# Apokleos/kata-xpu-device-plugin

Measured on NVIDIA H100. Metric: pci.ids parse GB/s (x1000 text + 2^20-key join); device lookups/s reported beside it, higher is better.
Workload: dtype u8

## Files before the change

### kata-xpu-device-plugin_b200/csrc/api.cu

```cuda
#include <algorithm>
#include <cstdlib>
#include <new>
#include <vector>

#include "internal.cuh"
#include "pciids5.cu"
#include "finalize.cuh"
#include "small.cuh"
#include "scan.cuh"

void kx_exchange_destroy(kxpu_ctx *ctx);

static const char *kx_err_names[] = {
    "ok", "invalid argument", "CUDA error", "no sm_90 GPU available", "output buffer too small",
    "table capacity exceeded", "NCCL / peer exchange unavailable or failed", "input outside the supported domain", "out of memory"};

extern "C" const char *kxpu_strerror(int32_t status) {
    int i = -status;
    if (i < 0 || i > 8) return "unknown status";
    return kx_err_names[i];
}

extern "C" const char *kxpu_last_error(kxpu_ctx *ctx) {
    if (!ctx) return "null ctx";
// ... 270 lines not shown
    t->dev.slots = (KxSlot *)(b + L.o_slots);
    t->dev.vendor_first = (unsigned long long *)(b + L.o_vfirst);
    t->dev.trunc = (unsigned long long *)(b + L.o_trunc);
    t->dev.counters = (uint32_t *)(b + L.o_counters);
    t->dev.cap = cap;
    t->dev.shift = t->shift;
    t->dev.max_keys = cap / 2;
    t->range_words = (unsigned long long *)(b + L.o_range);
    t->row_key = (uint32_t *)(b + L.o_row_key);
    t->row_line = (unsigned long long *)(b + L.o_row_line);
    t->row_anchor = (unsigned long long *)(b + L.o_row_anchor);
    t->row_name_off = (uint32_t *)(b + L.o_row_noff);
    t->row_name_len = (uint32_t *)(b + L.o_row_nlen);
    t->blob = b + L.o_blob;
    t->blob_cap = blob_cap;
    t->rows_cap = cap + 1;
    *out = t;
    return KXPU_OK;
}

void kx_table_release(kxpu_ctx *ctx, kxpu_table *t) {
    if (!t) return;
    if (t->arena.p) {
        if (ctx->pool.size() >= 4) {
            cudaStreamSynchronize(ctx->stream);
            cudaFree(ctx->pool.front().p);
            ctx->pool.erase(ctx->pool.begin());
        }
        arena_reset(ctx, t->arena);
        ctx->pool.push_back(t->arena);
    }
    delete t;
}

uint32_t kx_initial_blob_cap(kxpu_ctx *ctx, size_t n) {
    const uint32_t by_text = (uint32_t)std::min<size_t>(std::max<size_t>(n, 256), 4u << 20);
    return ctx->blob_hint > by_text ? ctx->blob_hint : by_text;
}

bool kx_grow_cap(uint32_t *cap, bool table_full) {
    if (*cap >= (1u << 28)) return false;
    const uint32_t sh = table_full ? 4u : 2u;
    *cap = (*cap >> (28u - sh)) ? (1u << 28) : (*cap << sh);
    return true;
}

void kx_note_table_size(kxpu_ctx *ctx, uint32_t nkeys, uint32_t blob_used, uint32_t blob_cap) {
    uint32_t ideal = 1u << 16;
    while (ideal < (1u << 28) && ideal / 2 < nkeys + nkeys / 8) ideal <<= 1;
    ctx->cap_hint = ideal;
    ctx->blob_hint = blob_cap > (4u << 20) && blob_used > (2u << 20) ? blob_cap : 0u;
}

int32_t kx_launch_parse(kxpu_ctx *ctx, kxpu_table *t, const uint8_t *d_text, size_t n, unsigned long long base,
                        unsigned long long carry_in, const KxXaHook *xa) {
    using namespace kxparse;
    const uint32_t num_chunks = (uint32_t)((n + CW - 1) / CW);
    kxparse5::Params5 P;
    memset(&P, 0, sizeof P);
    if (xa) { P.xa_on = 1; P.xa_done = xa->done; P.xa = xa->p; }
    if (num_chunks == 0) {
        if (xa) {
            P.tab = t->dev;
            P.task_ctas = 0;
            kxparse5::resolve_chunks_kernel<<<kxparse5::XA_CTAS, kxparse5::RES_WARPS * 32, 0, ctx->stream>>>(P);
            KX_LAUNCHED(ctx);
            KX_CUDA(ctx, cudaGetLastError());
        }
        return KXPU_OK;
    }
    P.text = d_text; P.n = n; P.base = base; P.num_chunks = num_chunks;
    P.tma_limit = n >= (size_t)STG_BYTES ? (uint32_t)((n - STG_BYTES) / CW) + 1u : 0u;
    static int per_sm = 0;
    const size_t smem = sizeof(kxparse5::WarpSmem5) * WARPS;
    if (per_sm == 0) {
        cudaOccupancyMaxActiveBlocksPerMultiprocessor(&per_sm, kxparse5::parse_kernel_v5, NT, smem);
        if (per_sm < 1) per_sm = 1;
    }
    const uint32_t wave_warps = (uint32_t)per_sm * ctx->sm_count * WARPS;
    P.rch = std::min<uint32_t>(std::max<uint32_t>(num_chunks / (wave_warps * 8u), 1u), kxparse5::RCH5_MAX);
    if (ctx->force_rch) P.rch = (uint32_t)ctx->force_rch;
    P.num_ranges = (num_chunks + P.rch - 1) / P.rch;
    P.range_state = t->range_words;
    P.range_carry = t->range_words + P.num_ranges;
    P.lead = (uint32_t *)(t->range_words + 2 * P.num_ranges);
    P.tasks = P.lead + P.num_ranges;
    P.tab = t->dev; P.carry_in = carry_in;
    uint32_t grid = (uint32_t)per_sm * ctx->sm_count;
    const uint32_t need = (P.num_ranges + WARPS - 1) / WARPS;
    if (grid > need) grid = need;
    {
        KxTimer tm(ctx, KXPU_T_PARSE);
        kxparse5::parse_kernel_v5<<<grid, NT, smem, ctx->stream>>>(P);
        KX_LAUNCHED(ctx);
    }
    {
        KxTimer tr(ctx, KXPU_T_RESOLVE);
        kxparse5::resolve_ranges_kernel<<<(P.num_ranges + 255u) / 256u, 256, 0, ctx->stream>>>(P);
        KX_LAUNCHED(ctx);
        const uint32_t rgrid = std::min<uint32_t>(4u * ctx->sm_count, (num_chunks + kxparse5::RES_WARPS - 1) / kxparse5::RES_WARPS);
        P.task_ctas = rgrid;
        kxparse5::resolve_chunks_kernel<<<rgrid + (xa ? kxparse5::XA_CTAS : 0u), kxparse5::RES_WARPS * 32, 0, ctx->stream>>>(P);
        KX_LAUNCHED(ctx);
    }
    KX_CUDA(ctx, cudaGetLastError());
    return KXPU_OK;
}

int32_t kx_launch_trunc(kxpu_ctx *ctx, kxpu_table *t, const uint8_t *d_text, size_t n, unsigned long long base) {
    kxparse::trunc_kernel<<<1, 1024, 0, ctx->stream>>>(d_text, n, base, t->dev.trunc, t->dev.counters);
    KX_LAUNCHED(ctx);
    KX_CUDA(ctx, cudaGetLastError());
    return KXPU_OK;
}

int32_t kx_launch_finalize(kxpu_ctx *ctx, kxpu_table *t, const uint8_t *d_text, size_t n, unsigned long long base,
                           const kxx::MinView *mv, const kxx::WaitSpec *wait, const KxSlabOut *slab) {
    kxparse::FinalizeParams F;
    memset(&F, 0, sizeof F);
    if (wait) F.wait = *wait;
    F.text = d_text; F.n = n; F.base = base; F.tab = t->dev;
    if (mv) F.mv = *mv;
    else { F.mv.a = t->dev.vendor_first; F.mv.stride = 0; F.mv.n = 1; F.mv.trunc1 = t->dev.trunc; }
    F.row_key = t->row_key; F.row_line = t->row_line; F.row_anchor = t->row_anchor;
    F.row_name_off = t->row_name_off; F.row_name_len = t->row_name_len;
    F.blob = t->blob; F.blob_cap = t->blob_cap;
    if (slab) {
        F.slab_rows = reinterpret_cast<kxx::SlabRow *>(slab->rows); F.slab_rows_cap = slab->rows_cap;
        F.blob = slab->blob; F.blob_cap = slab->blob_cap;
        F.tail = slab->tail;
    }
    KxTimer tm(ctx, KXPU_T_FINALIZE);
    F.scan_w = t->cap >= (1u << 19) ? 32u : 8u;
    if (ctx->force_scan_w) F.scan_w = (uint32_t)ctx->force_scan_w;
    const unsigned batches = (t->cap + 1 + F.scan_w - 1) / F.scan_w;
    const unsigned grid = std::min<unsigned>((batches + kxparse::SF_WARPS - 1) / kxparse::SF_WARPS, 8u * ctx->sm_count);
    kxparse::select_finalize_kernel<<<grid, kxparse::SF_WARPS * 32, 0, ctx->stream>>>(F);
    KX_LAUNCHED(ctx);
    KX_CUDA(ctx, cudaGetLastError());
    return KXPU_OK;
}

static unsigned join_ctas(kxpu_ctx *ctx, size_t n) { return (unsigned)std::min<size_t>((n + 255) / 256, (size_t)ctx->sm_count * 32); }

int32_t kx_launch_lookup(kxpu_ctx *ctx, kxpu_table *t, const uint32_t *d_keys, size_t n, int32_t *d_rows) {
    if (n == 0) return KXPU_OK;
    KxTimer tm(ctx, KXPU_T_LOOKUP);
    kxparse::lookup_kernel<<<join_ctas(ctx, n), 256, 0, ctx->stream>>>(d_keys, n, t->dev.slots, t->cap, t->shift, d_rows);
    KX_LAUNCHED(ctx);
    KX_CUDA(ctx, cudaGetLastError());
    return KXPU_OK;
}

static int32_t kx_launch_rows_names_join(kxpu_ctx *ctx, kxpu_table *t, const uint8_t *d_text, size_t n, const uint32_t *d_keys,
                                         size_t nq, int32_t *d_rows) {
    using namespace kxparse;
    FinalizeParams F;
    memset(&F, 0, sizeof F);
    F.text = d_text; F.n = n; F.base = 0; F.tab = t->dev;
    F.mv.a = t->dev.vendor_first; F.mv.stride = 0; F.mv.n = 1; F.mv.trunc1 = t->dev.trunc;
    F.row_key = t->row_key; F.row_line = t->row_line; F.row_anchor = t->row_anchor;
    F.row_name_off = t->row_name_off; F.row_name_len = t->row_name_len;
    F.blob = t->blob; F.blob_cap = t->blob_cap;
    KxTimer tm(ctx, KXPU_T_FINALIZE);
    select_rows_kernel<<<(t->cap + SF_WARPS * 32) / (SF_WARPS * 32), SF_WARPS * 32, 0, ctx->stream>>>(F);
    KX_LAUNCHED(ctx);
    const uint32_t want = (t->cap / 2 + SF_CTA_ROWS - 1) / SF_CTA_ROWS;
    const unsigned name_ctas = std::max<unsigned>(1u, std::min<unsigned>(want, 8u * ctx->sm_count));
    const unsigned grid = name_ctas + (nq ? join_ctas(ctx, nq) : 0u);
    names_join_kernel<<<grid, SF_WARPS * 32, 0, ctx->stream>>>(F, name_ctas, d_keys, nq, d_rows);
    KX_LAUNCHED(ctx);
    KX_CUDA(ctx, cudaGetLastError());
    return KXPU_OK;
}

struct KxJoin {
    const uint32_t *d_keys;
    size_t n;
    int32_t *d_rows;
    int32_t *h_rows;
    const uint8_t *src_text;
};

static void *kx_mapped_host(const void *p) {
    if (!p) return nullptr;
    cudaPointerAttributes at;
    if (cudaPointerGetAttributes(&at, p) != cudaSuccess) { cudaGetLastError(); return nullptr; }
    return at.type == cudaMemoryTypeHost ? at.devicePointer : nullptr;
}

static uint32_t small_text_chunks(kxpu_ctx *ctx) {
    if (ctx->small_chunks < 0) {
        int coop = 0, per_sm = 0;
        cudaDeviceGetAttribute(&coop, cudaDevAttrCooperativeLaunch, ctx->device);
        cudaFuncSetAttribute(kxsmall::small_load_kernel, cudaFuncAttributeMaxDynamicSharedMemorySize, kxparse::WARPS * kxparse::STG_BYTES);
        cudaOccupancyMaxActiveBlocksPerMultiprocessor(&per_sm, kxsmall::small_load_kernel, kxparse::NT, kxparse::WARPS * kxparse::STG_BYTES);
        cudaGetLastError();
        ctx->small_chunks = (coop && !ctx->no_small) ? per_sm * ctx->sm_count * kxparse::WARPS : 0;
    }
    return (uint32_t)ctx->small_chunks;
}

static int32_t launch_small(kxpu_ctx *ctx, kxpu_table *t, const uint8_t *d_text, size_t n, const KxJoin *join) {
    using namespace kxparse;
    kxsmall::SmallParams P;
    memset(&P, 0, sizeof P);
    P.text = d_text; P.n = n;
    P.num_chunks = (uint32_t)((n + CW - 1) / CW);
    P.tma_limit = n >= (size_t)STG_BYTES ? (uint32_t)((n - STG_BYTES) / CW) + 1u : 0u;
    P.state = t->range_words;
    FinalizeParams &F = P.F;
    F.text = d_text; F.n = n; F.base = 0; F.tab = t->dev;
    F.mv.a = t->dev.vendor_first; F.mv.stride = 0; F.mv.n = 1; F.mv.trunc1 = t->dev.trunc;
    F.row_key = t->row_key; F.row_line = t->row_line; F.row_anchor = t->row_anchor;
    F.row_name_off = t->row_name_off; F.row_name_len = t->row_name_len;
    F.blob = t->blob; F.blob_cap = t->blob_cap;
    if (join) { P.keys = join->d_keys; P.nq = join->n; P.rows_out = join->d_rows; }
    if (join && join->src_text) { P.text_src = join->src_text; P.h_ctl = ctx->h_ctl; }
    void *args[] = {&P};
    const unsigned grid = std::max<unsigned>((P.num_chunks + WARPS - 1) / WARPS, (unsigned)(ctx->small_chunks / WARPS));
    F.scan_w = 8u;
    while (F.scan_w < 32u && (size_t)(t->cap + 1 + F.scan_w - 1) / F.scan_w > (size_t)grid * SF_WARPS) F.scan_w *= 2u;
    if (ctx->force_scan_w) F.scan_w = (uint32_t)ctx->force_scan_w;
// ... 37 lines not shown
                fprintf(stderr, " %u: %lld/%lld/%lld/%lld |", c, tw[c * 4], tw[c * 4 + 1], tw[c * 4 + 2], tw[c * 4 + 3]);
            }
            const unsigned mid = wv[wv.size() / 2].second;
            fprintf(stderr, " median %u: %lld/%lld/%lld/%lld", mid, tw[mid * 4], tw[mid * 4 + 1], tw[mid * 4 + 2], tw[mid * 4 + 3]);
            const long long *tf = h.data() + (size_t)grid * 8 + (size_t)P.num_chunks * 4;
            static const char *fn[7] = {"scan", "rounds", "sync1+claim", "sync2", "names out+rows", "long lines", "shift+sync3"};
            fprintf(stderr, "\n   names phase per CTA (thread 0), cycles min/avg/max:");
            for (int k = 0; k < 7; k++) {
                long long mn = 1ll << 62, mx = 0, sum = 0, cnt = 0;
                for (unsigned b = 0; b < grid; b++) {
                    const long long t1 = tf[b * 8 + k], t0 = k ? tf[b * 8 + k - 1] : h[b * 8 + 4];
                    if (!t1 || !t0) continue;
                    const long long d = t1 - t0;
                    mn = std::min(mn, d); mx = std::max(mx, d); sum += d; cnt++;
                }
                if (cnt) fprintf(stderr, " %s %lld/%lld/%lld |", fn[k], mn, sum / cnt, mx);
            }
        }
        fprintf(stderr, "\n");
    }
    return KXPU_OK;
}

static int32_t kx_build_table_join(kxpu_ctx *ctx, const uint8_t *d_text, size_t n, kxpu_table **out, const KxJoin *join) {
    if ((reinterpret_cast<uintptr_t>(d_text) & 15u) != 0) {
        KX_SET_ERR(ctx, "device text pointer must be 16-byte aligned");
        return KXPU_E_INVALID;
    }
    if (n >= (1ull << 44)) return KXPU_E_UNSUPPORTED;
    uint32_t cap = ctx->cap_hint;
    while (cap > (1u << 16) && (size_t)cap / 2 > n / 6 + 1) cap >>= 1;
    uint32_t blob_cap = kx_initial_blob_cap(ctx, n);
    const uint32_t num_chunks = (uint32_t)((n + kxparse::CW - 1) / kxparse::CW);
    bool have_trunc = false;
    for (int attempt = 0; attempt < 12; attempt++) {
        kxpu_table *t = nullptr;
        int32_t rc = kx_table_acquire(ctx, cap, blob_cap, num_chunks, &t);
        if (rc != KXPU_OK) return rc;
        const bool small_path = num_chunks > 0 && num_chunks <= small_text_chunks(ctx) && !have_trunc;
        if (small_path) {
            rc = launch_small(ctx, t, d_text, n, join);
        } else {
            if (join && join->src_text && attempt == 0) cudaMemcpyAsync(const_cast<uint8_t *>(d_text), join->src_text, n, cudaMemcpyDefault, ctx->stream);
            rc = kx_launch_parse(ctx, t, d_text, n, 0, 0, nullptr);
            if (rc == KXPU_OK && have_trunc) rc = kx_launch_trunc(ctx, t, d_text, n, 0);
            if (rc == KXPU_OK)
                rc = join ? kx_launch_rows_names_join(ctx, t, d_text, n, join->d_keys, join->n, join->d_rows)
                          : kx_launch_rows_names_join(ctx, t, d_text, n, nullptr, 0, nullptr);
        }
        if (rc != KXPU_OK) { kx_table_release(ctx, t); return rc; }
        const bool zero_copy = small_path && join && join->src_text;
        if (!zero_copy) {
            if (join && join->h_rows && join->n) cudaMemcpyAsync(join->h_rows, join->d_rows, join->n * 4, cudaMemcpyDeviceToHost, ctx->stream);
            cudaMemcpyAsync(ctx->h_ctl, t->dev.counters, KX_C_COUNT * 4, cudaMemcpyDeviceToHost, ctx->stream);
        }
        cudaError_t e = cudaStreamSynchronize(ctx->stream);
        if (e != cudaSuccess) {
            KX_SET_ERR(ctx, "parse/finalize failed: %s", cudaGetErrorString(e));
            kx_table_release(ctx, t);
            return KXPU_E_CUDA;
        }
        const uint32_t *h = ctx->h_ctl;
        if (h[KX_C_OVERFLOW] || h[KX_C_NKEYS] > t->dev.max_keys) {
            kx_table_release(ctx, t);
            if (!kx_grow_cap(&cap, h[KX_C_OVERFLOW] != 0)) return KXPU_E_CAPACITY;
            continue;
        }
        if (h[KX_C_NEED_TRUNC] == 2u) {
            kx_table_release(ctx, t);
            have_trunc = true;
            continue;
        }
        if (h[KX_C_BLOB_OVERFLOW]) {
            kx_table_release(ctx, t);
            if ((size_t)blob_cap >= n) return KXPU_E_CAPACITY;
            blob_cap = (uint32_t)std::min<size_t>(std::max<size_t>(n, 256), (size_t)blob_cap * 8);
            continue;
        }
        t->n_rows = h[KX_C_NSEL];
        t->blob_used = h[KX_C_BLOB_CURSOR];
        kx_note_table_size(ctx, h[KX_C_NKEYS], t->blob_used, blob_cap);
        *out = t;
        return KXPU_OK;
    }
    return KXPU_E_CAPACITY;
}

extern "C" int32_t kxpu_pciids_load_device(kxpu_ctx *ctx, const void *d_text, size_t n, kxpu_table **out) {
    KX_ENTER(ctx);
    if (!out || (!d_text && n)) return KXPU_E_INVALID;
    kx_clear_timings(ctx);
    return kx_build_table_join(ctx, (const uint8_t *)d_text, n, out, nullptr);
}

extern "C" int32_t kxpu_pciids_join_device(kxpu_ctx *ctx, const void *d_text, size_t n, const uint32_t *d_keys, size_t nq,
                                           int32_t *d_rows_out, kxpu_table **out) {
    KX_ENTER(ctx);
    if (!out || (!d_text && n) || (nq && (!d_keys || !d_rows_out))) return KXPU_E_INVALID;
    kx_clear_timings(ctx);
    const KxJoin j{d_keys, nq, d_rows_out, nullptr, nullptr};
    return kx_build_table_join(ctx, (const uint8_t *)d_text, n, out, &j);
}

static int32_t stage_reserve(kxpu_ctx *ctx, size_t bytes) {
    if (bytes <= ctx->d_stage_bytes) return KXPU_OK;
    if (ctx->d_stage) {
        cudaStreamSynchronize(ctx->stream);
// ... 167 lines not shown
```

### kata-xpu-device-plugin_b200/csrc/common.cuh

```cuda
#pragma once
#include <cuda_runtime.h>
#include <stdint.h>
#include <stdio.h>
#include <string.h>

#include <mutex>
#include <vector>

#include "../../include/kxpu.h"

constexpr int KX_MAX_RANKS = 16;


struct KxArena {
    void *p = nullptr;
    size_t bytes = 0;
    uint32_t cap = 0, blob_cap = 0;
    size_t range_bytes = 0;
};

struct KxExchange;
struct kxpu_multi;

struct kxpu_ctx {
// ... 37 lines not shown
            KX_SET_ERR(ctx, "%s:%d %s -> %s", __FILE__, __LINE__, #call, cudaGetErrorString(e__)); \
            return KXPU_E_CUDA;                                                             \
        }                                                                                   \
    } while (0)

#define KX_LAUNCHED(ctx) ((ctx)->launches++)

struct KxTimer {
    kxpu_ctx *c;
    int idx;
    bool open = true;
    KxTimer(kxpu_ctx *ctx, int i) : c(ctx), idx(i) {
        open = c->stage_timing;
        if (open) cudaEventRecord(c->ev[2 * i], c->stream);
    }
    void stop() {
        if (open) { cudaEventRecord(c->ev[2 * idx + 1], c->stream); c->ev_used[idx] = true; open = false; }
    }
    ~KxTimer() { stop(); }
};

static inline void kx_clear_timings(kxpu_ctx *c) { memset(c->ev_used, 0, sizeof(c->ev_used)); }

unsigned long long *kx_scan_state(kxpu_ctx *ctx, size_t words);
uint32_t kx_next_epoch(kxpu_ctx *ctx);

int32_t kx_rule_drivers(kxpu_ctx *ctx, const kxpu_xpu_rule *rules, size_t n_rules, unsigned long long drv[][4]);

void kx_pcie_parse(cudaStream_t st, const kxpu_devrec *recs, const kxpu_pcipath *paths, uint32_t n, unsigned long long *chain,
                   uint8_t *clen);

struct KxScratch {
    kxpu_ctx *c;
    std::vector<void *> ptrs;
    explicit KxScratch(kxpu_ctx *ctx) : c(ctx) {}
    cudaError_t alloc(void **p, size_t bytes) {
        cudaError_t e = cudaMallocAsync(p, bytes ? bytes : 16, c->stream);
        if (e == cudaSuccess) ptrs.push_back(*p);
        else *p = nullptr;
        return e;
    }
    ~KxScratch() {
        for (void *p : ptrs) cudaFreeAsync(p, c->stream);
    }
};

#ifdef __CUDACC__
__device__ __forceinline__ uint32_t kx_lane() { return threadIdx.x & 31u; }

__device__ __forceinline__ void kx_fence_gpu() { asm volatile("fence.acq_rel.gpu;" ::: "memory"); }
__device__ __forceinline__ void kx_fence_sys() { asm volatile("fence.acq_rel.sys;" ::: "memory"); }

__device__ __forceinline__ uint32_t kx_hash(uint32_t key) { return key * 0x9E3779B1u; }
#endif
```

### kata-xpu-device-plugin_b200/csrc/finalize.cuh

```cuda
#pragma once
#include "exchange.cuh"
#include "parse_common.cuh"

namespace kxparse {

constexpr unsigned long long MAX_TOKEN = 65536ull;

__global__ void __launch_bounds__(1024) trunc_kernel(const uint8_t *__restrict__ text, unsigned long long n,
                                                      unsigned long long base, unsigned long long *trunc_out, uint32_t *counters) {
    __shared__ unsigned long long s_first[1024], s_last[1024], s_bad[1024];
    const unsigned long long per = (n + 1023ull) / 1024ull;
    const unsigned long long lo = per * threadIdx.x, hi = lo + per < n ? lo + per : n;
    unsigned long long first = KX_NO_OFF, last = KX_NO_OFF, bad = KX_NO_OFF;
    for (unsigned long long i = lo; i < hi; i++) {
        if (text[i] == (uint8_t)'\n') {
            if (first == KX_NO_OFF) first = i;
            else if (i - last - 1 >= MAX_TOKEN && bad == KX_NO_OFF) bad = last + 1;
            last = i;
        }
    }
    s_first[threadIdx.x] = first; s_last[threadIdx.x] = last; s_bad[threadIdx.x] = bad;
    __syncthreads();
    if (threadIdx.x == 0) {
        unsigned long long prev_nl = KX_NO_OFF;
// ... 386 lines not shown
        }
        SF_MARK(5);
        {
            const uint32_t rem = qn - nvalid;
            if (nvalid != 0u && rem != 0u) {
                SfEntry e;
                if (lane < rem) e = q[nvalid + lane];
                __syncwarp();
                if (lane < rem) q[lane] = e;
                __syncwarp();
            }
            qn = rem;
        }
        __syncthreads();
        SF_MARK(6);
        if (!more) break;
    }
}

__global__ void __launch_bounds__(SF_WARPS * 32, 8) select_finalize_kernel(const FinalizeParams F) {
    kxx::wait_flags_cta(F.wait);
    select_finalize_body(F, F.scan_w);
    if (F.tail.on) {
        __syncthreads();
        if (threadIdx.x == 0) {
            kx_fence_sys();
            const uint32_t prev = atomicAdd(F.tail.done, 1u);
            if (prev == gridDim.x - 1u) {
                *F.tail.done = 0u;
                kx_fence_gpu();
                const volatile uint32_t *c = F.tab.counters;
                const uint32_t n_sel = c[KX_C_NSEL], blob_used = c[KX_C_BLOB_CURSOR];
                const bool over = c[KX_C_BLOB_OVERFLOW] || n_sel > F.tail.rows_cap || blob_used > F.tail.blob_cap;
                kxx::SlabHeader h;
                memset(&h, 0, sizeof h);
                h.n_rows = over ? 0u : n_sel;
                h.blob_bytes = over ? 0u : blob_used;
                h.status = over ? kxx::XS_SLAB_OVERFLOW : 0u;
                if (c[KX_C_OVERFLOW]) h.status |= kxx::XS_GROW | kxx::XS_FULL;
                if (c[KX_C_NKEYS] > F.tab.max_keys) h.status |= kxx::XS_GROW;
                h.nkeys = c[KX_C_NKEYS];
                *F.tail.header = h;
                kx_fence_sys();
                for (int k = 0; k < F.tail.tg.n; k++) *reinterpret_cast<volatile uint32_t *>(F.tail.tg.region[k] + F.tail.o_flag) = F.tail.epoch;
            }
        }
    }
}

constexpr uint32_t SF_CTA_ROWS = SF_WARPS * SF_BATCH;

__global__ void __launch_bounds__(SF_WARPS * 32) select_rows_kernel(const FinalizeParams F) {
    __shared__ uint32_t s_cnt[SF_WARPS], s_row0;
    if (sf_stand_back(F)) return;
    const uint32_t lane = threadIdx.x & 31u, wl = threadIdx.x >> 5;
    const uint32_t slot = blockIdx.x * blockDim.x + threadIdx.x;
    uint32_t key = 0;
    unsigned long long line = 0, anchor = 0;
    const bool valid = slot <= F.tab.cap && sf_slot_valid(F, slot, kxx::min_view_trunc(F.mv), key, line, anchor);
    const uint32_t vm = __ballot_sync(0xffffffffu, valid);
    if (lane == 0) s_cnt[wl] = (uint32_t)__popc(vm);
    __syncthreads();
    if (threadIdx.x == 0) {
        uint32_t rows = 0, blob0;
#pragma unroll
        for (int k = 0; k < SF_WARPS; k++) rows += s_cnt[k];
        sf_cta_claim(F, rows, 0u, s_row0, blob0);
    }
    __syncthreads();
    if (valid) {
        uint32_t row = s_row0 + (uint32_t)__popc(vm & ((1u << lane) - 1u));
        for (uint32_t k = 0; k < wl; k++) row += s_cnt[k];
        F.tab.slots[slot].row = (int32_t)row;
        F.row_key[row] = key; F.row_line[row] = line; F.row_anchor[row] = anchor;
    }
}

__device__ __forceinline__ void names_body(const FinalizeParams &F, uint32_t ctas) {
    __shared__ __align__(16) uint8_t s_raw[SF_WARPS][4][SF_WIN + 16];
    __shared__ uint8_t s_name[SF_WARPS][SF_BATCH][SF_WIN];
    __shared__ uint32_t s_bytes[SF_WARPS], s_blob0;
    const uint32_t lane = threadIdx.x & 31u, wl = threadIdx.x >> 5;
    const uint32_t n_rows = F.tab.counters[KX_C_NSEL];
    for (uint32_t c0 = blockIdx.x * SF_CTA_ROWS; c0 < n_rows; c0 += ctas * SF_CTA_ROWS) {
        const uint32_t r0 = c0 + wl * (uint32_t)SF_BATCH;
        const uint32_t nvalid = r0 < n_rows ? min(n_rows - r0, (uint32_t)SF_BATCH) : 0u;
        uint32_t my_len, slow_m;
        sf_name_batch(F, lane < nvalid ? F.row_line[r0 + lane] : 0ull, nvalid, s_raw[wl], s_name[wl], my_len, slow_m);
        const uint32_t len_r = (lane < nvalid && !((slow_m >> lane) & 1u)) ? my_len : 0u;
        const uint32_t incl = sf_incl_scan(len_r);
        const uint32_t wtot = __shfl_sync(0xffffffffu, incl, 31);
        if (lane == 0) s_bytes[wl] = wtot;
        __syncthreads();
        if (threadIdx.x == 0) {
            uint32_t bytes = 0, row0;
#pragma unroll
            for (int k = 0; k < SF_WARPS; k++) bytes += s_bytes[k];
            sf_cta_claim(F, 0u, bytes, row0, s_blob0);
        }
        __syncthreads();
        uint32_t blob0 = s_blob0;
        for (uint32_t k = 0; k < wl; k++) if (blob0 != 0xFFFFFFFFu) blob0 += s_bytes[k];
        const bool room = blob0 != 0xFFFFFFFFu;
        const uint32_t off_r = room ? blob0 + incl - len_r : 0u, len_w = room ? len_r : 0u;
        sf_names_out(F, s_name[wl], nvalid, len_w, off_r);
        if (lane < nvalid && !((slow_m >> lane) & 1u)) { F.row_name_off[r0 + lane] = off_r; F.row_name_len[r0 + lane] = len_w; }
        __syncwarp();
        for (uint32_t sm = slow_m; sm; sm &= sm - 1u) {
            const uint32_t r = (uint32_t)__ffs((int)sm) - 1u;
            uint32_t name_off, name_len;
            sf_long_name(F, F.row_line[r0 + r], &s_name[wl][0][0], name_off, name_len);
            if (lane == 0) { F.row_name_off[r0 + r] = name_off; F.row_name_len[r0 + r] = name_len; }
            __syncwarp();
        }
        __syncthreads();
    }
}

__global__ void __launch_bounds__(SF_WARPS * 32, 8) names_join_kernel(const FinalizeParams F, uint32_t name_ctas,
                                                                       const uint32_t *__restrict__ keys, size_t nq,
                                                                       int32_t *__restrict__ rows_out) {
    if (blockIdx.x < name_ctas) {
        names_body(F, name_ctas);
        return;
    }
    const size_t stride = (size_t)(gridDim.x - name_ctas) * blockDim.x;
    for (size_t i = (size_t)(blockIdx.x - name_ctas) * blockDim.x + threadIdx.x; i < nq; i += stride)
        rows_out[i] = table_probe(F.tab.slots, F.tab.cap, F.tab.shift, keys[i]);
}

__global__ void __launch_bounds__(256) lookup_kernel(const uint32_t *__restrict__ keys, size_t n, const KxSlot *__restrict__ slots,
                                                      uint32_t cap, uint32_t shift, int32_t *__restrict__ rows_out) {
    size_t i = (size_t)blockIdx.x * blockDim.x + threadIdx.x;
    const size_t stride = (size_t)gridDim.x * blockDim.x;
    for (; i < n; i += stride) rows_out[i] = table_probe(slots, cap, shift, keys[i]);
}

__global__ void __launch_bounds__(256) name_len_kernel(const int32_t *__restrict__ rows, size_t n,
                                                        const uint32_t *__restrict__ row_name_len, uint32_t n_rows,
                                                        uint32_t *__restrict__ lens) {
    size_t i = (size_t)blockIdx.x * blockDim.x + threadIdx.x;
    if (i < n) {
        int32_t r = rows[i];
        lens[i] = (r >= 0 && (uint32_t)r < n_rows) ? row_name_len[r] : 0u;
    }
}
__global__ void __launch_bounds__(256) name_copy_kernel(const int32_t *__restrict__ rows, size_t n,
                                                         const uint32_t *__restrict__ row_name_off,
                                                         const uint32_t *__restrict__ row_name_len, uint32_t n_rows,
                                                         const uint8_t *__restrict__ blob,
                                                         const uint32_t *__restrict__ offsets, uint8_t *__restrict__ out,
                                                         size_t cap) {
    size_t i = ((size_t)blockIdx.x * blockDim.x + threadIdx.x) >> 3;
    uint32_t sub = threadIdx.x & 7u;
    if (i >= n) return;
    int32_t r = rows[i];
    if (r < 0 || (uint32_t)r >= n_rows) return;
    uint32_t len = row_name_len[r], src = row_name_off[r], dst = offsets[i];
    if ((size_t)dst + len > cap) return;
    for (uint32_t k = sub; k < len; k += 8u) out[dst + k] = blob[src + k];
}

__global__ void __launch_bounds__(256) arena_reset_kernel(uint4 *ff, size_t n_ff16, uint32_t *counters) {
    const size_t i = (size_t)blockIdx.x * blockDim.x + threadIdx.x;
    const size_t stride = (size_t)gridDim.x * blockDim.x;
    for (size_t k = i; k < n_ff16; k += stride) ff[k] = make_uint4(0xffffffffu, 0xffffffffu, 0xffffffffu, 0xffffffffu);
    if (i < KX_C_COUNT) counters[i] = 0u;
}

}
```

### kata-xpu-device-plugin_b200/csrc/pciids5.cu

```cuda
#pragma once
#include "exchange.cuh"
#include "parse_common.cuh"

namespace kxparse5 {

using namespace kxparse;

constexpr int CPC5 = 3;
constexpr int STAGES5 = 2;
constexpr int CTAS5 = 2;
constexpr int COPY5 = CPC5 * CW + TRAIL;
constexpr int RCH5_MAX = CPC5 * STAGES5;
constexpr int RES_WARPS = 8;

struct WarpSmem5 {
    alignas(16) uint8_t stage[STAGES5][COPY5];
    alignas(8) unsigned long long bar[STAGES5];
};

struct Params5 {
    const uint8_t *text;
    unsigned long long n, base;
    uint32_t num_chunks;
    uint32_t tma_limit;
// ... 30 lines not shown
    }
}

__device__ __forceinline__ uint32_t tops_of(uint32_t lp, uint32_t mm) {
    uint32_t tm = 0;
    while (mm) {
        const uint32_t bit = mm & (0u - mm);
        mm ^= bit;
        const uint32_t c0 = lds8(lp + (31u - (uint32_t)__clz((int)bit)));
        if (c0 != 9u && c0 != 35u) tm |= bit;
    }
    return tm;
}

__device__ __forceinline__ void tops_of2(uint32_t lp0, uint32_t m0, uint32_t m1, uint32_t &t0, uint32_t &t1) {
    t0 = t1 = 0;
    while (m0 | m1) {
        const uint32_t b0 = m0 & (0u - m0), b1 = m1 & (0u - m1);
        m0 ^= b0;
        m1 ^= b1;
        const uint32_t c0 = lds8(lp0 + (31u - (uint32_t)__clz((int)b0)));
        const uint32_t c1 = lds8(lp0 + (uint32_t)HALF + (31u - (uint32_t)__clz((int)b1)));
        if (c0 != 9u && c0 != 35u) t0 |= b0;
        if (c1 != 9u && c1 != 35u) t1 |= b1;
    }
}

__device__ __forceinline__ uint32_t devs_of(uint32_t lp, uint32_t mm) {
    uint32_t km = 0;
    while (mm) {
        const uint32_t bit = mm & (0u - mm);
        mm ^= bit;
        const uint32_t a = lp + (31u - (uint32_t)__clz((int)bit));
        if (lds8(a) == 9u && lds8(a + 1u) != 9u) km |= bit;
    }
    return km;
}

__global__ void __launch_bounds__(NT, CTAS5) parse_kernel_v5(const Params5 P) {
    extern __shared__ __align__(128) uint8_t smem_raw[];
    WarpSmem5 *W = reinterpret_cast<WarpSmem5 *>(smem_raw);
    uint32_t lane = threadIdx.x & 31u;
    const uint32_t w = threadIdx.x >> 5;
    asm volatile("" : "+r"(lane));
    const uint32_t lt_mask = (1u << lane) - 1u;

    if (lane == 0) {
        for (int s = 0; s < STAGES5; s++) mbar_init(&W[w].bar[s], 1);
        asm volatile("fence.mbarrier_init.release.cluster;" ::: "memory");
    }
    uint32_t tk = 0;
    if (lane == 0) tk = atomicAdd(&P.tab.counters[KX_C_TICKET], 1u);
    uint32_t r = __shfl_sync(0xffffffffu, tk, 0);
    if (r >= P.num_ranges) return;

    uint32_t a_stage0 = smem_u32(smem_raw) + w * (uint32_t)sizeof(WarpSmem5);
    asm volatile("" : "+r"(a_stage0));
    const uint32_t a_bar0 = a_stage0 + (uint32_t)offsetof(WarpSmem5, bar);

    uint32_t k7f = 0x7f7f7f7fu, k0a = 0x0a0a0a0au, k80 = 0x80808080u;
    asm volatile("" : "+r"(k7f), "+r"(k0a), "+r"(k80));

    const unsigned long long pol = l2_evict_first_policy();
    const uint32_t rch = P.rch;
    auto copy_chunks = [](uint32_t cnt, uint32_t k) -> uint32_t {
        return cnt - k * (uint32_t)CPC5 < (uint32_t)CPC5 ? cnt - k * (uint32_t)CPC5 : (uint32_t)CPC5;
    };
    auto issue = [&](uint32_t g0, uint32_t m, uint32_t s) {
        if (g0 + m - 1u < P.tma_limit) {
            mbar_expect_tx_a(a_bar0 + 8u * s, m * (uint32_t)CW + (uint32_t)TRAIL);
            tma_load_a(a_stage0 + s * (uint32_t)COPY5, P.text + (unsigned long long)g0 * CW, m * (uint32_t)CW + (uint32_t)TRAIL, a_bar0 + 8u * s, pol);
        }
    };

    uint32_t phase_bits = 0, s = 0;
    uint32_t nfresh = 0;
    for (;;) {
        uint32_t tk2 = 0;
        if (lane == 0) tk2 = atomicAdd(&P.tab.counters[KX_C_TICKET], 1u);
        uint32_t rc_x = 0, rc_g = 0;
        if (r == 0u) {
            rc_x = LS_PUB | (((P.carry_in & CV_HAS_TOP) && (P.carry_in & CV_VOK)) ? (LS_TOP | LS_VOK) : 0u);
            rc_g = 0xffffffffu;
        }
        uint32_t lead = r == 0u ? 0u : rch;
        const bool table_dead = *reinterpret_cast<volatile uint32_t *>(&P.tab.counters[KX_C_OVERFLOW]) != 0u;
        const uint32_t gb = r * rch;
        const uint32_t cnt = P.num_chunks - gb < rch ? P.num_chunks - gb : rch;
        const uint32_t ncp = (cnt + (uint32_t)CPC5 - 1u) / (uint32_t)CPC5;
        if (lane == 0) {
            for (uint32_t j = 0; j < (uint32_t)STAGES5 && j < ncp; j++) issue(gb + j * (uint32_t)CPC5, copy_chunks(cnt, j), (s + j) % (uint32_t)STAGES5);
        }
        for (uint32_t k = 0; k < ncp; k++) {
            const uint32_t g0 = gb + k * (uint32_t)CPC5, m = copy_chunks(cnt, k);
            const bool by_tma = g0 + m - 1u < P.tma_limit;
            if (by_tma) {
                const uint32_t bar = a_bar0 + 8u * s, par = (phase_bits >> s) & 1u;
                while (!mbar_try_a(bar, par)) {
                }
                phase_bits ^= 1u << s;
            }
            for (uint32_t j = 0; j < m; j++) {
                const uint32_t i = k * (uint32_t)CPC5 + j;
                const uint32_t g = g0 + j;
                const uint32_t st = a_stage0 + s * (uint32_t)COPY5 + j * (uint32_t)CW;
                const unsigned long long cbase = P.base + (unsigned long long)g * CW;
                uint32_t n_rel = CW + 1;
// ... 92 lines not shown
                    const uint32_t l1 = __shfl_sync(0xffffffffu, linfo1, bal1 ? 31 - __clz((int)bal1) : 0);
                    const uint32_t last0 = bal0 ? l0 : base_info;
                    const uint32_t cin0 = s0 ? x0 : base_info;
                    const uint32_t cin1 = s1 ? x1 : last0;
                    last1 = bal1 ? l1 : last0;
                    if (cin0 != P_NONE && (cin0 >> 31))
                        fold_lines(P.tab, st, cbase, pre0, lane * 32u + 1u, ((cin0 >> 15) & 0xffffu) << 16, cbase + (cin0 & 0x7fffu), nfresh);
                    if (cin1 != P_NONE && (cin1 >> 31))
                        fold_lines(P.tab, st, cbase, pre1, (uint32_t)HALF + lane * 32u + 1u, ((cin1 >> 15) & 0xffffu) << 16, cbase + (cin1 & 0x7fffu), nfresh);
                    const uint32_t hw0 = cin0 == P_NONE ? pre0 : 0u;
                    const uint32_t hw1 = cin1 == P_NONE ? pre1 : 0u;
                    if (rc_x & LS_VOK) {
                        uint32_t key_hi = ((rc_x >> 12) & 0xffffu) << 16;
                        unsigned long long anchor = P.base + (unsigned long long)rc_g * CW + (rc_x & 0xfffu);
                        if (rc_g == 0xffffffffu) {
                            key_hi = ((uint32_t)(P.carry_in >> 44) & 0xffffu) << 16;
                            anchor = P.carry_in & CV_ANCHOR_MASK;
                        }
                        if ((hw0 | hw1) != 0u && P.tab.vendor_first[key_hi >> 16] >= anchor) {
                            fold_lines(P.tab, st, cbase, hw0, lane * 32u + 1u, key_hi, anchor, nfresh);
                            fold_lines(P.tab, st, cbase, hw1, (uint32_t)HALF + lane * 32u + 1u, key_hi, anchor, nfresh);
                        }
                    }
                    flush_fresh(P.tab, nfresh);
                }
                if (last1 != P_NONE) {
                    if (rc_x == 0u) lead = i + 1u;
                    rc_x = LS_PUB | LS_TOP | ((last1 >> 31) ? LS_VOK : 0u) | (((last1 >> 15) & 0xffffu) << 12) | (last1 & 0xfffu);
                    rc_g = g;
                }
                if ((bal0 | bal1) == 0u && n_rel > (uint32_t)CW && __reduce_or_sync(0xffffffffu, rawnl) == 0u && lane == 0)
                    atomicOr(&P.tab.counters[KX_C_LONGLINE_HINT], 1u);
                __syncwarp();
            }

            if (lane == 0 && k + (uint32_t)STAGES5 < ncp) issue(gb + (k + (uint32_t)STAGES5) * (uint32_t)CPC5, copy_chunks(cnt, k + (uint32_t)STAGES5), s);
            s = s == (uint32_t)STAGES5 - 1u ? 0u : s + 1u;
        }
        if (lane == 0) {
            unsigned long long v = ST_NONE;
            if (rc_x != 0u) {
                if (rc_g == 0xffffffffu)
                    v = ST_PREFIX | P.carry_in;
                else
                    v = ST_PREFIX | CV_HAS_TOP | ((rc_x & LS_VOK) ? CV_VOK : 0ull) | ((unsigned long long)((rc_x >> 12) & 0xffffu) << 44) |
                        ((P.base + (unsigned long long)rc_g * CW + (rc_x & 0xfffu)) & CV_ANCHOR_MASK);
            }
            P.range_state[r] = v;
            P.lead[r] = lead < cnt ? lead : cnt;
        }
        r = __shfl_sync(0xffffffffu, tk2, 0);
        if (r >= P.num_ranges) break;
    }
}

constexpr uint32_t XA_CTAS = 64;

__global__ void __launch_bounds__(256) resolve_ranges_kernel(const Params5 P) {
    const uint32_t rr = blockIdx.x * blockDim.x + threadIdx.x;
    const uint32_t lane = threadIdx.x & 31u;
    const uint32_t rr0 = rr - lane;
    if (rr0 >= P.num_ranges) return;
    const bool live = rr < P.num_ranges;
    const uint32_t nlead = live ? P.lead[rr] : 0u;
    const unsigned long long own = live ? P.range_state[rr] : ST_NONE;
    const uint32_t pm = __ballot_sync(0xffffffffu, (own & ST_MASK) == ST_PREFIX);
    const uint32_t below = pm & ((1u << lane) - 1u);
    const unsigned long long from_warp = __shfl_sync(0xffffffffu, own, below ? 31 - __clz((int)below) : 0);
    unsigned long long warp_in = 0;
    const uint32_t first_p = pm ? (uint32_t)__ffs((int)pm) - 1u : 32u;
    const bool want = __any_sync(0xffffffffu, nlead != 0u && lane <= first_p);
    if (want) {
        long long q0 = (long long)rr0 - 32;
        for (;;) {
            const long long q = q0 + lane;
            const unsigned long long sv = q >= 0 ? P.range_state[q] : (q == -1 ? (ST_PREFIX | P.carry_in) : ST_NONE);
            const uint32_t m = __ballot_sync(0xffffffffu, (sv & ST_MASK) == ST_PREFIX);
            if (m) {
                warp_in = __shfl_sync(0xffffffffu, sv, 31 - __clz((int)m));
                break;
            }
            q0 -= 32;
        }
    }
    const unsigned long long carry = (below ? from_warp : warp_in) & ~ST_MASK;
    const bool alive = nlead != 0u && (carry & CV_HAS_TOP) && (carry & CV_VOK) &&
                       P.tab.vendor_first[(uint32_t)(carry >> 44) & 0xffffu] >= (carry & CV_ANCHOR_MASK);
    const uint32_t mine = alive ? nlead : 0u;
    uint32_t incl = mine;
#pragma unroll
    for (int d = 1; d < 32; d <<= 1) {
        const uint32_t y = __shfl_up_sync(0xffffffffu, incl, d);
        if (lane >= (uint32_t)d) incl += y;
    }
    const uint32_t tot = __shfl_sync(0xffffffffu, incl, 31);
    uint32_t at0 = 0;
    if (lane == 0 && tot) at0 = atomicAdd(&P.tab.counters[KX_C_DEFER], tot);
    at0 = __shfl_sync(0xffffffffu, at0, 0);
    if (!alive) return;
    P.range_carry[rr] = carry;
    const uint32_t at = at0 + incl - mine;
    for (uint32_t j = 0; j < nlead; j++) P.tasks[at + j] = rr * P.rch + j;
}

__global__ void __launch_bounds__(RES_WARPS * 32) resolve_chunks_kernel(const Params5 P) {
    __shared__ __align__(16) uint8_t stg[RES_WARPS][STG_BYTES];
    __shared__ __align__(8) unsigned long long bars[RES_WARPS];
    __shared__ uint16_t plist[RES_WARPS][704];
    if (blockIdx.x >= P.task_ctas) {
        kxx::xa_push_slice(P.xa, (blockIdx.x - P.task_ctas) * blockDim.x + threadIdx.x, XA_CTAS * blockDim.x);
        __syncthreads();
        if (threadIdx.x == 0) {
            kx_fence_sys();
            const uint32_t prev = atomicAdd(P.xa_done, 1u);
            if (prev == XA_CTAS - 1u) {
                *P.xa_done = 0u;
                kx_fence_sys();
                kxx::xa_finish(P.xa);
            }
        }
        return;
    }
    const uint32_t lane = threadIdx.x & 31u, w = threadIdx.x >> 5;
    const uint32_t lt_mask = (1u << lane) - 1u;
    uint32_t k7f = 0x7f7f7f7fu, k0a = 0x0a0a0a0au, k80 = 0x80808080u;
    asm volatile("" : "+r"(k7f), "+r"(k0a), "+r"(k80));
    const uint32_t st = smem_u32(stg[w]), bar = smem_u32(&bars[w]);
    if (lane == 0) {
        mbar_init(&bars[w], 1);
        asm volatile("fence.mbarrier_init.release.cluster;" ::: "memory");
    }
    __syncwarp();
    const unsigned long long pol = l2_evict_first_policy();
    const uint32_t n_tasks = P.tab.counters[KX_C_DEFER];
    uint32_t par = 0, nfresh = 0;
    const bool small_tab = P.tab.cap <= (1u << 20);
    uint32_t it = 0;
    for (uint32_t t = blockIdx.x * RES_WARPS + w; t < n_tasks; t += P.task_ctas * RES_WARPS, it++) {
        if ((it & 3u) == 0u && *reinterpret_cast<volatile uint32_t *>(&P.tab.counters[KX_C_OVERFLOW]) != 0u) break;
        const uint32_t gg = P.tasks[t];
        uint32_t n_rel = CW + 1;
        if (gg < P.tma_limit) {
            if (lane == 0) {
                mbar_expect_tx_a(bar, STG_BYTES);
                tma_load_a(st, P.text + (unsigned long long)gg * CW, STG_BYTES, bar, pol);
            }
            while (!mbar_try_a(bar, par)) {
            }
            par ^= 1u;
        } else {
            n_rel = stage_chunk_manual(P.text, P.n, gg, lane, stg[w]);
        }
        const unsigned long long cc = P.range_carry[gg / P.rch];
        const uint32_t key_hi = ((uint32_t)(cc >> 44) & 0xffffu) << 16;
        const unsigned long long anchor = cc & CV_ANCHOR_MASK;
        uint32_t kh[2], th[2], rawnl;
        chunk_masks(st, lane, n_rel, k7f, k0a, k80, kh, th, rawnl);
        const uint32_t bal0 = __ballot_sync(0xffffffffu, th[0] != 0u);
        const uint32_t bal1 = __ballot_sync(0xffffffffu, th[1] != 0u);
        const uint32_t pre0 = kh[0] & ~th[0] & (th[0] ? (th[0] & (0u - th[0])) - 1u : 0xffffffffu);
        const uint32_t pre1 = kh[1] & ~th[1] & (th[1] ? (th[1] & (0u - th[1])) - 1u : 0xffffffffu);
        const unsigned long long cbase = P.base + (unsigned long long)gg * CW;
        const uint32_t m0 = (bal0 & lt_mask) == 0u ? pre0 : 0u;
        const uint32_t m1 = (bal0 == 0u && (bal1 & lt_mask) == 0u) ? pre1 : 0u;
        const uint32_t mine = (uint32_t)__popc(m0) + (uint32_t)__popc(m1);
        uint32_t incl = mine;
#pragma unroll
        for (int d = 1; d < 32; d <<= 1) {
            const uint32_t y = __shfl_up_sync(0xffffffffu, incl, d);
            if (lane >= (uint32_t)d) incl += y;
        }
        const uint32_t total = __shfl_sync(0xffffffffu, incl, 31);
        {
            uint32_t idx = incl - mine;
            for (uint32_t m = m0; m; m &= m - 1u) plist[w][idx++] = (uint16_t)(lane * 32u + 1u + (uint32_t)__ffs((int)m) - 1u);
            for (uint32_t m = m1; m; m &= m - 1u) plist[w][idx++] = (uint16_t)((uint32_t)HALF + lane * 32u + 1u + (uint32_t)__ffs((int)m) - 1u);
        }
        __syncwarp();
        if (small_tab) {
            for (uint32_t i = lane; i < total; i += 64u) {
                uint32_t d0, d1 = 0;
                const uint32_t p0 = plist[w][i], p1 = i + 32u < total ? plist[w][i + 32u] : 0u;
                bool v0 = hex4_swar(lds32_unaligned(st + p0 + 1u), d0);
                bool v1 = i + 32u < total && hex4_swar(lds32_unaligned(st + p1 + 1u), d1);
                uint32_t q0 = p0, q1 = p1;
                if (!v0 && v1) { d0 = d1; q0 = p1; v0 = true; v1 = false; }
// ... 16 lines not shown
```

### kata-xpu-device-plugin_b200/csrc/table.cuh

```cuda
#pragma once
#include "common.cuh"

#define KX_EMPTY_KEY 0xFFFFFFFFu
#define KX_NO_OFF 0xFFFFFFFFFFFFFFFFull

#define KX_C_TICKET 0
#define KX_C_DEFER 1
#define KX_C_GRIDBAR 2
#define KX_C_NKEYS 32
#define KX_C_NSEL 33
#define KX_C_BLOB_CURSOR 64
#define KX_C_OVERFLOW 96
#define KX_C_LONGLINE_HINT 97
#define KX_C_NROWS 98
#define KX_C_BLOB_OVERFLOW 99
#define KX_C_NEED_TRUNC 100
#define KX_C_XSTATUS 101
#define KX_C_XROWS 102
#define KX_C_XBLOB 103
#define KX_C_XMAXKEYS 104
#define KX_C_COUNT 128

struct __align__(32) KxSlot {
    uint32_t key;
    int32_t row;
    unsigned long long min_line;
    unsigned long long min_anchor;
    unsigned long long spare;
};

struct KxTableDev {
    KxSlot *slots;
    unsigned long long *vendor_first;
    uint32_t *counters;
    unsigned long long *trunc;
    uint32_t cap;
    uint32_t shift;
    uint32_t max_keys;
};
```

Baseline: 2687.

## Chain parse/resolve/finalize kernels with PDL and write counters to host from device

```diff
diff --git a/kata-xpu-device-plugin_b200/csrc/api.cu b/kata-xpu-device-plugin_b200/csrc/api.cu
--- a/kata-xpu-device-plugin_b200/csrc/api.cu
+++ b/kata-xpu-device-plugin_b200/csrc/api.cu
@@ -346,6 +346,23 @@
     ctx->blob_hint = blob_cap > (4u << 20) && blob_used > (2u << 20) ? blob_cap : 0u;
 }
 
+template <typename... KArgs, typename... Args>
+static cudaError_t kx_launch_pdl(kxpu_ctx *ctx, void (*kernel)(KArgs...), unsigned grid, unsigned block, size_t smem, Args &&...args) {
+    cudaLaunchAttribute at[1];
+    at[0].id = cudaLaunchAttributeProgrammaticStreamSerialization;
+    at[0].val.programmaticStreamSerializationAllowed = 1;
+    cudaLaunchConfig_t cfg = {};
+    cfg.gridDim = dim3(grid);
+    cfg.blockDim = dim3(block);
+    cfg.dynamicSmemBytes = smem;
+    cfg.stream = ctx->stream;
+    cfg.attrs = at;
+    cfg.numAttrs = 1;
+    const cudaError_t e = cudaLaunchKernelEx(&cfg, kernel, std::forward<Args>(args)...);
+    KX_LAUNCHED(ctx);
+    return e;
+}
+
 int32_t kx_launch_parse(kxpu_ctx *ctx, kxpu_table *t, const uint8_t *d_text, size_t n, unsigned long long base,
                         unsigned long long carry_in, const KxXaHook *xa) {
     using namespace kxparse;
@@ -390,12 +407,10 @@
     }
     {
         KxTimer tr(ctx, KXPU_T_RESOLVE);
-        kxparse5::resolve_ranges_kernel<<<(P.num_ranges + 255u) / 256u, 256, 0, ctx->stream>>>(P);
-        KX_LAUNCHED(ctx);
+        KX_CUDA(ctx, kx_launch_pdl(ctx, kxparse5::resolve_ranges_kernel, (P.num_ranges + 255u) / 256u, 256u, 0, P));
         const uint32_t rgrid = std::min<uint32_t>(4u * ctx->sm_count, (num_chunks + kxparse5::RES_WARPS - 1) / kxparse5::RES_WARPS);
         P.task_ctas = rgrid;
-        kxparse5::resolve_chunks_kernel<<<rgrid + (xa ? kxparse5::XA_CTAS : 0u), kxparse5::RES_WARPS * 32, 0, ctx->stream>>>(P);
-        KX_LAUNCHED(ctx);
+        KX_CUDA(ctx, kx_launch_pdl(ctx, kxparse5::resolve_chunks_kernel, rgrid + (xa ? kxparse5::XA_CTAS : 0u), kxparse5::RES_WARPS * 32u, 0, P));
     }
     KX_CUDA(ctx, cudaGetLastError());
     return KXPU_OK;
@@ -457,12 +472,11 @@
     F.row_name_off = t->row_name_off; F.row_name_len = t->row_name_len;
     F.blob = t->blob; F.blob_cap = t->blob_cap;
     KxTimer tm(ctx, KXPU_T_FINALIZE);
-    select_rows_kernel<<<(t->cap + SF_WARPS * 32) / (SF_WARPS * 32), SF_WARPS * 32, 0, ctx->stream>>>(F);
-    KX_LAUNCHED(ctx);
+    KX_CUDA(ctx, kx_launch_pdl(ctx, select_rows_kernel, (t->cap + SF_WARPS * 32) / (SF_WARPS * 32), SF_WARPS * 32u, 0, F));
     const uint32_t want = (t->cap / 2 + SF_CTA_ROWS - 1) / SF_CTA_ROWS;
     const unsigned name_ctas = std::max<unsigned>(1u, std::min<unsigned>(want, 8u * ctx->sm_count));
     const unsigned grid = name_ctas + (nq ? join_ctas(ctx, nq) : 0u);
-    names_join_kernel<<<grid, SF_WARPS * 32, 0, ctx->stream>>>(F, name_ctas, d_keys, nq, d_rows);
+    names_join_kernel<<<grid, SF_WARPS * 32, 0, ctx->stream>>>(F, name_ctas, d_keys, nq, d_rows, ctx->h_ctl);
     KX_LAUNCHED(ctx);
     KX_CUDA(ctx, cudaGetLastError());
     return KXPU_OK;
@@ -606,7 +620,7 @@
         const bool zero_copy = small_path && join && join->src_text;
         if (!zero_copy) {
             if (join && join->h_rows && join->n) cudaMemcpyAsync(join->h_rows, join->d_rows, join->n * 4, cudaMemcpyDeviceToHost, ctx->stream);
-            cudaMemcpyAsync(ctx->h_ctl, t->dev.counters, KX_C_COUNT * 4, cudaMemcpyDeviceToHost, ctx->stream);
+            if (small_path) cudaMemcpyAsync(ctx->h_ctl, t->dev.counters, KX_C_COUNT * 4, cudaMemcpyDeviceToHost, ctx->stream);
         }
         cudaError_t e = cudaStreamSynchronize(ctx->stream);
         if (e != cudaSuccess) {
diff --git a/kata-xpu-device-plugin_b200/csrc/common.cuh b/kata-xpu-device-plugin_b200/csrc/common.cuh
--- a/kata-xpu-device-plugin_b200/csrc/common.cuh
+++ b/kata-xpu-device-plugin_b200/csrc/common.cuh
@@ -113,4 +113,7 @@
 __device__ __forceinline__ void kx_fence_sys() { asm volatile("fence.acq_rel.sys;" ::: "memory"); }
 
 __device__ __forceinline__ uint32_t kx_hash(uint32_t key) { return key * 0x9E3779B1u; }
+
+__device__ __forceinline__ void kx_pdl_wait() { asm volatile("griddepcontrol.wait;" ::: "memory"); }
+__device__ __forceinline__ void kx_pdl_trigger() { asm volatile("griddepcontrol.launch_dependents;" ::: "memory"); }
 #endif
diff --git a/kata-xpu-device-plugin_b200/csrc/finalize.cuh b/kata-xpu-device-plugin_b200/csrc/finalize.cuh
--- a/kata-xpu-device-plugin_b200/csrc/finalize.cuh
+++ b/kata-xpu-device-plugin_b200/csrc/finalize.cuh
@@ -462,6 +462,7 @@
 
 __global__ void __launch_bounds__(SF_WARPS * 32) select_rows_kernel(const FinalizeParams F) {
     __shared__ uint32_t s_cnt[SF_WARPS], s_row0;
+    kx_pdl_wait();
     if (sf_stand_back(F)) return;
     const uint32_t lane = threadIdx.x & 31u, wl = threadIdx.x >> 5;
     const uint32_t slot = blockIdx.x * blockDim.x + threadIdx.x;
@@ -529,14 +530,24 @@
 
 __global__ void __launch_bounds__(SF_WARPS * 32, 8) names_join_kernel(const FinalizeParams F, uint32_t name_ctas,
                                                                        const uint32_t *__restrict__ keys, size_t nq,
-                                                                       int32_t *__restrict__ rows_out) {
-    if (blockIdx.x < name_ctas) {
-        names_body(F, name_ctas);
+                                                                       int32_t *__restrict__ rows_out, uint32_t *h_ctl) {
+    __shared__ uint32_t s_last;
+    if (blockIdx.x >= name_ctas) {
+        const size_t stride = (size_t)(gridDim.x - name_ctas) * blockDim.x;
+        for (size_t i = (size_t)(blockIdx.x - name_ctas) * blockDim.x + threadIdx.x; i < nq; i += stride)
+            rows_out[i] = table_probe(F.tab.slots, F.tab.cap, F.tab.shift, keys[i]);
         return;
     }
-    const size_t stride = (size_t)(gridDim.x - name_ctas) * blockDim.x;
-    for (size_t i = (size_t)(blockIdx.x - name_ctas) * blockDim.x + threadIdx.x; i < nq; i += stride)
-        rows_out[i] = table_probe(F.tab.slots, F.tab.cap, F.tab.shift, keys[i]);
+    names_body(F, name_ctas);
+    __syncthreads();
+    if (threadIdx.x == 0) {
+        kx_fence_gpu();
+        s_last = atomicAdd(&F.tab.counters[KX_C_DONE], 1u) == name_ctas - 1u;
+        if (s_last) kx_fence_gpu();
+    }
+    __syncthreads();
+    if (s_last && h_ctl)
+        for (uint32_t i = threadIdx.x; i < (uint32_t)KX_C_COUNT; i += blockDim.x) h_ctl[i] = __ldcg(&F.tab.counters[i]);
 }
 
 __global__ void __launch_bounds__(256) lookup_kernel(const uint32_t *__restrict__ keys, size_t n, const KxSlot *__restrict__ slots,
diff --git a/kata-xpu-device-plugin_b200/csrc/pciids5.cu b/kata-xpu-device-plugin_b200/csrc/pciids5.cu
--- a/kata-xpu-device-plugin_b200/csrc/pciids5.cu
+++ b/kata-xpu-device-plugin_b200/csrc/pciids5.cu
@@ -106,7 +106,10 @@
     uint32_t tk = 0;
     if (lane == 0) tk = atomicAdd(&P.tab.counters[KX_C_TICKET], 1u);
     uint32_t r = __shfl_sync(0xffffffffu, tk, 0);
-    if (r >= P.num_ranges) return;
+    if (r >= P.num_ranges) {
+        kx_pdl_trigger();
+        return;
+    }
 
     uint32_t a_stage0 = smem_u32(smem_raw) + w * (uint32_t)sizeof(WarpSmem5);
     asm volatile("" : "+r"(a_stage0));
@@ -305,6 +308,7 @@
         r = __shfl_sync(0xffffffffu, tk2, 0);
         if (r >= P.num_ranges) break;
     }
+    kx_pdl_trigger();
 }
 
 constexpr uint32_t XA_CTAS = 64;
@@ -313,6 +317,8 @@
     const uint32_t rr = blockIdx.x * blockDim.x + threadIdx.x;
     const uint32_t lane = threadIdx.x & 31u;
     const uint32_t rr0 = rr - lane;
+    kx_pdl_trigger();
+    kx_pdl_wait();
     if (rr0 >= P.num_ranges) return;
     const bool live = rr < P.num_ranges;
     const uint32_t nlead = live ? P.lead[rr] : 0u;
@@ -360,7 +366,9 @@
     __shared__ __align__(16) uint8_t stg[RES_WARPS][STG_BYTES];
     __shared__ __align__(8) unsigned long long bars[RES_WARPS];
     __shared__ uint16_t plist[RES_WARPS][704];
+    kx_pdl_trigger();
     if (blockIdx.x >= P.task_ctas) {
+        kx_pdl_wait();
         kxx::xa_push_slice(P.xa, (blockIdx.x - P.task_ctas) * blockDim.x + threadIdx.x, XA_CTAS * blockDim.x);
         __syncthreads();
         if (threadIdx.x == 0) {
@@ -385,6 +393,7 @@
     }
     __syncwarp();
     const unsigned long long pol = l2_evict_first_policy();
+    kx_pdl_wait();
     const uint32_t n_tasks = P.tab.counters[KX_C_DEFER];
     uint32_t par = 0, nfresh = 0;
     const bool small_tab = P.tab.cap <= (1u << 20);
diff --git a/kata-xpu-device-plugin_b200/csrc/table.cuh b/kata-xpu-device-plugin_b200/csrc/table.cuh
--- a/kata-xpu-device-plugin_b200/csrc/table.cuh
+++ b/kata-xpu-device-plugin_b200/csrc/table.cuh
@@ -7,6 +7,7 @@
 #define KX_C_TICKET 0
 #define KX_C_DEFER 1
 #define KX_C_GRIDBAR 2
+#define KX_C_DONE 3
 #define KX_C_NKEYS 32
 #define KX_C_NSEL 33
 #define KX_C_BLOB_CURSOR 64
```

Measured after the change: 2719, median of 6. About the same (+1.2%).
